# jenicek/mdir

Measured on AMD Instinct MI355X. Metric: queries/sec, exact full ranking (rOxford5k+1M-distractor shape, 2048-d fp32); mAP-medium alongside, higher is better.
Workload: dtype f32

## Files before the change

mdir_amd/csrc/mdx_rank.hip:

```cpp
#include <atomic>

#include "mdx_common.h"

#ifndef MDX_SORT_NT
#define MDX_SORT_NT 1
#endif

namespace mdx {

#ifndef MDX_SORT_ITEMS
#define MDX_SORT_ITEMS 8
#endif
constexpr int SORT_ITEMS = MDX_SORT_ITEMS;
#ifndef MDX_SORT_WAVES
#define MDX_SORT_WAVES 8
#endif
constexpr int SORT_WAVES = MDX_SORT_WAVES;
constexpr int SORT_THREADS = 64 * SORT_WAVES;
constexpr int SORT_TILE = SORT_THREADS * SORT_ITEMS;
constexpr int SUB_TILE = 64 * SORT_ITEMS;
constexpr int RADIX = 256;

__device__ __forceinline__ void bitonic_sort_lds(uint64_t *buf, int P, int tid, int nthreads)
{
    for (int size = 2; size <= P; size <<= 1)
        for (int stride = size >> 1; stride > 0; stride >>= 1) {
            for (int t = tid; t < (P >> 1); t += nthreads) {
                const int i = 2 * t - (t & (stride - 1)), j = i + stride;
                const uint64_t a = buf[i], b = buf[j];
                if ((a > b) == ((i & size) == 0)) {
                    buf[i] = b;
                    buf[j] = a;
                }
            }
            __syncthreads();
        }
}

enum { FMT_SCORES = 0, FMT_KV = 1, FMT_A = 2, FMT_B = 3, FMT_C = 4, FMT_RANKS = 5 };

constexpr int MAX_SEG = 32;
struct NoSeg { static constexpr bool HAS = false; };
struct SegTable {
    static constexpr bool HAS = true;
    const float *p[MAX_SEG];
    int64_t start[MAX_SEG + 1];
    int nseg;
    uint32_t inv_w;
};

struct SegHit { const float *p; int64_t s0, s1; int g; };

__device__ __forceinline__ SegHit seg_find(const SegTable &t, int64_t i)
{
    int g = (int)__umulhi((uint32_t)i, t.inv_w);
    if (g > t.nseg - 1) g = t.nseg - 1;
    SegHit h = {t.p[g], t.start[g], t.start[g + 1], g};
    while (i >= h.s1 && g + 1 < t.nseg) { ++g; h.p = t.p[g]; h.s0 = h.s1; h.s1 = t.start[g + 1]; }
    while (i < h.s0 && g > 0) { --g; h.p = t.p[g]; h.s1 = h.s0; h.s0 = t.start[g]; }
    h.g = g;
    return h;
}

struct SegPair { const uint32_t *a, *b; int64_t cut; bool ok; };

__device__ __forceinline__ SegPair seg_pair(const SegTable &t, const SegHit &h, int64_t q, int64_t tile_end)
{
    SegPair r = {nullptr, nullptr, h.s1, false};
    if (h.g + 1 >= t.nseg) return r;
    const int64_t n0 = t.start[h.g + 1], n1 = t.start[h.g + 2];
    if (tile_end > n1) return r;
    r.a = (const uint32_t *)(h.p + q * (h.s1 - h.s0) - h.s0);
    r.b = (const uint32_t *)(t.p[h.g + 1] + q * (n1 - n0) - n0);
    r.ok = true;
    return r;
}

__device__ __forceinline__ const float *seg_elem(const SegTable &t, int64_t q, int64_t i)
{
    const SegHit h = seg_find(t, i);
    return h.p + q * (h.s1 - h.s0) + (i - h.s0);
}

constexpr int HIST_COPIES = 8;

template <int SRC, typename SEGT = NoSeg>
__global__ __launch_bounds__(SORT_THREADS) void sort_hist_kernel(const float *__restrict__ scores,
                                                                 const void *__restrict__ src, int64_t n,
                                                                 int64_t stride, int nblk, int shift,
                                                                 uint32_t *__restrict__ block_hist, SEGT seg)
{
    static_assert(SORT_ITEMS == 8, "a lane takes 8 elements of a tile");
    constexpr bool FIRST = SRC == FMT_SCORES;
    __shared__ uint32_t h[HIST_COPIES][RADIX + 1];
    const int tid = threadIdx.x, copy = tid & (HIST_COPIES - 1);
    const int64_t q = FIRST ? (int64_t)gridDim.y - 1 - blockIdx.y : (int64_t)blockIdx.y;
    const int64_t b0 = FIRST ? (int64_t)gridDim.x - 1 - blockIdx.x : (int64_t)blockIdx.x;
    for (int e = tid; e < HIST_COPIES * (RADIX + 1); e += SORT_THREADS) (&h[0][0])[e] = 0;
    uint32_t d[SORT_ITEMS];
    int64_t first[2];
    if (SRC == FMT_A || SRC == FMT_B) {
        const int64_t i = b0 * SORT_TILE + tid * 8;
        first[0] = i;
        first[1] = i + 4;
        if (SRC == FMT_A) {
            typedef uint16_t u16x8 __attribute__((ext_vector_type(8)));
            u16x8 w = {0, 0, 0, 0, 0, 0, 0, 0};
            if (i < n) w = *(const u16x8 *)((const uint16_t *)src + q * stride + i);
#pragma unroll
            for (int j = 0; j < 8; ++j) d[j] = w[j] & 255u;
        } else {
            typedef uint8_t u8x8 __attribute__((ext_vector_type(8)));
            u8x8 w = {0, 0, 0, 0, 0, 0, 0, 0};
            if (i < n) w = *(const u8x8 *)((const uint8_t *)src + q * stride + i);
#pragma unroll
            for (int j = 0; j < 8; ++j) d[j] = w[j];
        }
    } else {
        typedef uint32_t u32x4u __attribute__((ext_vector_type(4), aligned(4)));
        const uint32_t *p = FIRST ? (const uint32_t *)scores + q * n : (const uint32_t *)src + q * stride;
        u32x4u w[2];
#pragma unroll
        for (int v = 0; v < 2; ++v) {
            first[v] = b0 * SORT_TILE + (v * SORT_THREADS + tid) * 4;
            w[v] = u32x4u{0u, 0u, 0u, 0u};
        }
        bool straddles = false;
        const int64_t tile_end = (b0 + 1) * SORT_TILE < n ? (b0 + 1) * SORT_TILE : n;
        SegHit h = {nullptr, 0, 0, 0};
        if constexpr (FIRST && SEGT::HAS) {
            h = seg_find(seg, b0 * SORT_TILE);
            straddles = tile_end > h.s1;
            p = (const uint32_t *)(h.p + q * (h.s1 - h.s0) - h.s0);
        }
        if (straddles) {
            if constexpr (SEGT::HAS) {
                const SegPair pr = seg_pair(seg, h, q, tile_end);
                if (pr.ok) {
#pragma unroll
                    for (int v = 0; v < 2; ++v) {
                        const int64_t i0 = first[v];
                        if (i0 + 4 <= pr.cut) w[v] = *(const u32x4u *)(pr.a + i0);
                        else if (i0 >= pr.cut && i0 + 4 <= tile_end) w[v] = *(const u32x4u *)(pr.b + i0);
                        else {
#pragma unroll
                            for (int j = 0; j < 4; ++j)
                                if (i0 + j < tile_end) w[v][j] = (i0 + j < pr.cut ? pr.a : pr.b)[i0 + j];
                        }
                    }
                } else {
#pragma unroll
                    for (int v = 0; v < 2; ++v)
#pragma unroll
                        for (int j = 0; j < 4; ++j)
                            if (first[v] + j < n) w[v][j] = *(const uint32_t *)seg_elem(seg, q, first[v] + j);
                }
            }
        } else if ((b0 + 1) * SORT_TILE <= n) {
#pragma unroll
            for (int v = 0; v < 2; ++v) w[v] = *(const u32x4u *)(p + first[v]);
        } else {
#pragma unroll
            for (int v = 0; v < 2; ++v)
#pragma unroll
                for (int j = 0; j < 4; ++j)
                    if (first[v] + j < n) w[v][j] = p[first[v] + j];
        }
#pragma unroll
        for (int v = 0; v < 2; ++v)
#pragma unroll
            for (int j = 0; j < 4; ++j) d[v * 4 + j] = ((FIRST ? desc_key(__uint_as_float(w[v][j])) : w[v][j]) >> shift) & 255u;
    }
    __syncthreads();
#pragma unroll
    for (int r = 0; r < SORT_ITEMS; ++r)
        if (first[r / 4] + (r % 4) < n) atomicAdd(&h[copy][d[r]], 1u);
    __syncthreads();
    for (int e = tid; e < RADIX; e += SORT_THREADS) {
        uint32_t tot = 0;
#pragma unroll
        for (int w = 0; w < HIST_COPIES; ++w) tot += h[w][e];
        block_hist[(q * nblk + b0) * RADIX + e] = tot;
    }
}

constexpr int SCAN_GROUPS = 32, SCAN_DIGITS = 32;

__global__ __launch_bounds__(SCAN_GROUPS * SCAN_DIGITS) void sort_scan_kernel(uint32_t *__restrict__ block_hist,
                                                                              int nblk,
                                                                              uint32_t *__restrict__ digit_tot)
{
    __shared__ uint32_t part[SCAN_GROUPS][SCAN_DIGITS + 1];
    const int dl = threadIdx.x & (SCAN_DIGITS - 1), g = threadIdx.x / SCAN_DIGITS;
    const int d = blockIdx.x * SCAN_DIGITS + dl;
    const int64_t q = blockIdx.y;
    const int per = (nblk + SCAN_GROUPS - 1) / SCAN_GROUPS;
    const int b0 = g * per < nblk ? g * per : nblk, b1 = (b0 + per) < nblk ? (b0 + per) : nblk;
    uint32_t *p = block_hist + q * nblk * RADIX + d;
    uint32_t sum = 0;
    constexpr int KEEP = 8;
    uint32_t kept[KEEP];
    const bool keep = per <= KEEP;
    if (keep) {
#pragma unroll
        for (int u = 0; u < KEEP; ++u) {
            kept[u] = (b0 + u) < b1 ? p[(int64_t)(b0 + u) * RADIX] : 0u;
            sum += kept[u];
        }
    } else {
        for (int b = b0; b < b1; ++b) sum += p[(int64_t)b * RADIX];
    }
    part[g][dl] = sum;
    __syncthreads();
    uint32_t run = 0;
    for (int k = 0; k < g; ++k) run += part[k][dl];
    if (g == SCAN_GROUPS - 1) digit_tot[q * RADIX + d] = run + sum;
    if (keep) {
#pragma unroll
        for (int u = 0; u < KEEP; ++u)
            if ((b0 + u) < b1) {
                p[(int64_t)(b0 + u) * RADIX] = run;
                run += kept[u];
            }
        return;
    }
    int b = b0;
    for (; b + 8 <= b1; b += 8) {
        uint32_t c[8];
#pragma unroll
        for (int u = 0; u < 8; ++u) c[u] = p[(int64_t)(b + u) * RADIX];
#pragma unroll
        for (int u = 0; u < 8; ++u) {
            p[(int64_t)(b + u) * RADIX] = run;
            run += c[u];
        }
    }
    for (; b < b1; ++b) {
        const uint32_t c = p[(int64_t)b * RADIX];
        p[(int64_t)b * RADIX] = run;
        run += c;
    }
}

template <int IN, int OUT, bool ARANK, typename SEGT = NoSeg>
__global__ __launch_bounds__(SORT_THREADS, (SORT_WAVES >= 16 ? 8 : (3 * SORT_WAVES) / 4)) void sort_scatter_kernel(
    const float *__restrict__ scores, const uint32_t *__restrict__ w_in, const void *__restrict__ h_in,
    uint32_t *__restrict__ w_out, void *__restrict__ h_out, int64_t *__restrict__ ranks,
    float *__restrict__ top_scores, int64_t n, int64_t stride, int nblk, int shift,
    const uint32_t *__restrict__ block_hist, const uint32_t *__restrict__ digit_tot, int64_t id_offset,
    int64_t klimit, SEGT seg)
{
    constexpr bool FIRST = IN == FMT_SCORES, LAST = OUT == FMT_RANKS;
    constexpr bool VAL_IN_KEY = IN == FMT_C;
    __shared__ uint32_t dtot[RADIX];
    __shared__ uint32_t wcnt[SORT_WAVES][RADIX];
    __shared__ uint32_t gdelta[RADIX];
    __shared__ uint32_t scan[RADIX];
    __shared__ uint32_t skey[SORT_TILE];
    __shared__ uint32_t sval[SORT_TILE];
    const int tid = threadIdx.x, lane = tid & 63, wave = tid >> 6;
    const int64_t q = FIRST ? (int64_t)blockIdx.y : (int64_t)gridDim.y - 1 - blockIdx.y;
    int64_t b = blockIdx.x;
#ifndef MDX_SORT_NO_XCD
    {
        const int qn = nblk / 8, rn = nblk % 8, x = (int)(blockIdx.x % 8), k = (int)(blockIdx.x / 8);
        b = (x < rn ? (int64_t)x * (qn + 1) : (int64_t)rn * (qn + 1) + (int64_t)(x - rn) * qn) + k;
    }
#endif
    if (!FIRST) b = (int64_t)nblk - 1 - b;
    for (int e = tid; e < SORT_WAVES * RADIX; e += SORT_THREADS) (&wcnt[0][0])[e] = 0;
    __syncthreads();

    const int64_t base = q * n;
    const int64_t row = q * stride;
    const int64_t tile0 = b * SORT_TILE;
    const int tile_n = (int)((n - tile0) < SORT_TILE ? (n - tile0) : SORT_TILE);
    const int sub = wave * SUB_TILE + lane;
    uint32_t key[SORT_ITEMS], val[SORT_ITEMS], pos[SORT_ITEMS];
    uint32_t gbase = 0, qtot = 0;
    if (tid < RADIX) {
        gbase = block_hist[(q * nblk + b) * RADIX + tid];
        qtot = digit_tot[q * RADIX + tid];
    }
    if (FIRST) {
        typedef uint32_t u32x4u __attribute__((ext_vector_type(4), aligned(4)));
        const uint32_t *src = (const uint32_t *)scores + base + tile0;
        bool straddles = false;
        SegHit sh = {nullptr, 0, 0, 0};
        if constexpr (SEGT::HAS) {
            sh = seg_find(seg, tile0);
            straddles = tile0 + tile_n > sh.s1;
            src = (const uint32_t *)(sh.p + q * (sh.s1 - sh.s0) + (tile0 - sh.s0));
        }
        if (straddles) {
            if constexpr (SEGT::HAS) {
                const SegPair pr = seg_pair(seg, sh, q, tile0 + tile_n);
                if (pr.ok) {
                    const uint32_t *pa = pr.a + tile0, *pb = pr.b + tile0;
                    const int cut = (int)(pr.cut - tile0);
                    for (int e = tid; e < tile_n; e += SORT_THREADS) skey[e] = desc_key(__uint_as_float((e < cut ? pa : pb)[e]));
                } else {
                    for (int e = tid; e < tile_n; e += SORT_THREADS) skey[e] = desc_key(*seg_elem(seg, q, tile0 + e));
                }
            }
        } else if (tile_n == SORT_TILE) {
            u32x4u w[SORT_ITEMS / 4];
#pragma unroll
            for (int v = 0; v < SORT_ITEMS / 4; ++v) w[v] = *(const u32x4u *)(src + (v * SORT_THREADS + tid) * 4);
#pragma unroll
            for (int v = 0; v < SORT_ITEMS / 4; ++v)
#pragma unroll
                for (int j = 0; j < 4; ++j) skey[(v * SORT_THREADS + tid) * 4 + j] = desc_key(__uint_as_float(w[v][j]));
        } else {
            for (int e = tid; e < tile_n; e += SORT_THREADS) skey[e] = desc_key(__uint_as_float(src[e]));
        }
        __syncthreads();
#pragma unroll
        for (int r = 0; r < SORT_ITEMS; ++r) {
            key[r] = (sub + r * 64) < tile_n ? skey[sub + r * 64] : 0xFFFFFFFFu;
            val[r] = (uint32_t)tile0 + (uint32_t)(sub + r * 64);
        }
    } else {
        const uint32_t *wt = w_in + row + tile0;
        const uint8_t *ht = (const uint8_t *)h_in + (row + tile0) * (IN == FMT_KV ? 4 : IN == FMT_A ? 2 : 1);
        uint32_t w[SORT_ITEMS], hh[SORT_ITEMS];
#pragma unroll
        for (int r = 0; r < SORT_ITEMS; ++r) {
            const int e = min(sub + r * 64, tile_n - 1);
            w[r] = wt[e];
            hh[r] = 0;
            if (IN == FMT_KV) hh[r] = ((const uint32_t *)ht)[e];
            if (IN == FMT_A) hh[r] = ((const uint16_t *)ht)[e];
            if (IN == FMT_B) hh[r] = ht[e];
        }
#pragma unroll
        for (int r = 0; r < SORT_ITEMS; ++r) {
            const bool valid = (sub + r * 64) < tile_n;
            if (IN == FMT_KV) {
                key[r] = valid ? w[r] : 0xFFFFFFFFu;
                val[r] = hh[r];
            } else {
                const uint32_t k = IN == FMT_C ? w[r] : ((w[r] & 0xFF000000u) | (hh[r] << (IN == FMT_A ? 8 : 16)));
                key[r] = valid ? k : 0xFFFFFFFFu;
                val[r] = w[r] & 0x00FFFFFFu;
            }
        }
    }
    if (tid < RADIX) {
        gdelta[tid] = gbase;
        dtot[tid] = qtot;
    }
    uint32_t *mycnt = wcnt[wave];
    if (ARANK) {
#pragma unroll
        for (int r = 0; r < SORT_ITEMS; ++r) {
            pos[r] = 0;
            if ((sub + r * 64) < tile_n)
                pos[r] = __hip_atomic_fetch_add(&mycnt[(key[r] >> shift) & 255u], 1u, __ATOMIC_RELAXED,
                                                __HIP_MEMORY_SCOPE_WORKGROUP);
        }
    } else {
#pragma unroll
        for (int r = 0; r < SORT_ITEMS; ++r) {
            const bool valid = (sub + r * 64) < tile_n;
            const uint32_t d = (key[r] >> shift) & 255u;
            uint32_t dlo = 0, dhi = 0;
#pragma unroll
            for (int bit = 0; bit < 8; ++bit) {
                int32_t sel = __builtin_amdgcn_sbfe((int32_t)d, bit, 1);
                asm("" : "+v"(sel));
                const uint64_t m = __builtin_amdgcn_ballot_w64(sel < 0);
                dlo = __builtin_amdgcn_bitop3_b32(dlo, (uint32_t)m, (uint32_t)sel, 0xF6);
                dhi = __builtin_amdgcn_bitop3_b32(dhi, (uint32_t)(m >> 32), (uint32_t)sel, 0xF6);
            }
            const uint64_t vmask = __builtin_amdgcn_ballot_w64(valid);
            const uint32_t plo = (uint32_t)vmask & ~dlo, phi = (uint32_t)(vmask >> 32) & ~dhi;
            const uint32_t rank = __builtin_amdgcn_mbcnt_hi(phi, __builtin_amdgcn_mbcnt_lo(plo, 0u));
            const uint32_t cnt = __popc(plo) + __popc(phi);
            const uint32_t old = mycnt[d];
            __builtin_amdgcn_wave_barrier();
            if (valid && rank == 0) mycnt[d] = old + cnt;
            __builtin_amdgcn_wave_barrier();
            pos[r] = old + rank;
        }
    }
    __syncthreads();
    if (tid < RADIX) {
        uint32_t run = 0;
#pragma unroll
        for (int w = 0; w < SORT_WAVES; ++w) {
            const uint32_t c = wcnt[w][tid];
            wcnt[w][tid] = run;
            run += c;
        }
        scan[tid] = run;
    }
    __syncthreads();
    if (wave == 0) {
        const uint32_t t0 = scan[4 * lane], t1 = scan[4 * lane + 1], t2 = scan[4 * lane + 2],
                       t3 = scan[4 * lane + 3];
        const uint32_t g0 = dtot[4 * lane], g1 = dtot[4 * lane + 1], g2 = dtot[4 * lane + 2],
                       g3 = dtot[4 * lane + 3];
        const uint32_t mine = t0 + t1 + t2 + t3, gmine = g0 + g1 + g2 + g3;
        const uint32_t inc = wave_inclusive_sum(mine), ginc = wave_inclusive_sum(gmine);
        const uint32_t ex = inc - mine, gex = ginc - gmine;
        const uint32_t toff[4] = {ex, ex + t0, ex + t0 + t1, ex + t0 + t1 + t2};
        const uint32_t goff[4] = {gex, gex + g0, gex + g0 + g1, gex + g0 + g1 + g2};
#pragma unroll
        for (int k = 0; k < 4; ++k) {
            const int dgt = 4 * lane + k;
            scan[dgt] = toff[k];
            gdelta[dgt] += goff[k] - toff[k];
        }
    }
    __syncthreads();
#pragma unroll
    for (int r = 0; r < SORT_ITEMS; ++r) {
        if ((sub + r * 64) >= tile_n) continue;
        const uint32_t d = (key[r] >> shift) & 255u;
        const uint32_t lp = scan[d] + mycnt[d] + pos[r];
        skey[lp] = key[r];
        if (!VAL_IN_KEY) sval[lp] = val[r];
    }
    __syncthreads();
    constexpr bool OFF32 = IN == FMT_C;
    char *const wrow = (char *)(w_out + row), *const hrow = (char *)h_out + row * (OUT == FMT_KV ? 4 : OUT == FMT_A ? 2 : 1);
#pragma unroll
    for (int r = 0; r < SORT_ITEMS; ++r) {
        const int i = r * SORT_THREADS + tid;
        if (i >= tile_n) continue;
        const uint32_t k = skey[i], v = VAL_IN_KEY ? (k & 0x00FFFFFFu) : sval[i];
        const uint32_t dst32 = gdelta[(k >> shift) & 255u] + (uint32_t)i;
        if (LAST) {
            const int64_t dst = (int64_t)dst32;
            if (dst < klimit) {
                if (ranks) {
                    int64_t *dstp = OFF32 ? (int64_t *)((char *)(ranks + q * klimit) + (dst32 << 3)) : ranks + q * klimit + dst;
#if MDX_SORT_NT
                    __builtin_nontemporal_store((int64_t)v + id_offset, dstp);
#else
                    *dstp = (int64_t)v + id_offset;
#endif
                }
                if (top_scores) top_scores[q * klimit + dst] = scores[base + v];
            }
        } else if (OUT == FMT_KV) {
            w_out[row + (int64_t)dst32] = k;
            ((uint32_t *)h_out)[row + (int64_t)dst32] = v;
        } else {
            *(uint32_t *)(wrow + (dst32 << 2)) = (k & 0xFF000000u) | v;
            if (OUT == FMT_A) *(uint16_t *)(hrow + (dst32 << 1)) = (uint16_t)(k >> 8);
            if (OUT == FMT_B) *(uint8_t *)(hrow + dst32) = (uint8_t)(k >> 16);
        }
    }
}

constexpr int CNT_TILE = 4096;
constexpr int CNT_ITEMS = CNT_TILE / 256;

constexpr int CNTB_REFS = 256;

__global__ __launch_bounds__(256) void rank_count_bsearch_kernel(
    const float *__restrict__ scores, int64_t n, int64_t id_offset,
    const float *__restrict__ ref_scores, const int64_t *__restrict__ ref_ids,
    const int64_t *__restrict__ offsets, unsigned long long *__restrict__ cnt, int nblk)
{
    constexpr int CNT_COPIES = 8;
    __shared__ uint64_t sref[CNTB_REFS];
    __shared__ uint32_t histc[CNT_COPIES][CNTB_REFS + 1];
    __shared__ uint32_t hist[CNTB_REFS + 1];
    __shared__ uint32_t wsum[4];
    const int tid = threadIdx.x, lane = tid & 63, copy = tid & (CNT_COPIES - 1);
    const int64_t q = blockIdx.y;
    const int64_t lo = offsets[q], hi = offsets[q + 1];
    for (int64_t r0 = lo; r0 < hi; r0 += CNTB_REFS) {
        const int nref = (int)((hi - r0) < CNTB_REFS ? (hi - r0) : CNTB_REFS);
        int P = 2;
        while (P < nref) P <<= 1;
        __syncthreads();
        uint64_t mine = ~0ull;
        if (tid < nref) {
            const int64_t id = ref_ids[r0 + tid];
            const uint32_t idc = id < 0 ? 0u : (id > 0xFFFFFFFFll ? 0xFFFFFFFFu : (uint32_t)id);
            mine = ((uint64_t)desc_key(ref_scores[r0 + tid]) << 32) | idc;
        }
        sref[tid] = mine;
        for (int e = tid; e < CNT_COPIES * (CNTB_REFS + 1); e += 256) (&histc[0][0])[e] = 0;
        __syncthreads();
        bitonic_sort_lds(sref, CNTB_REFS, tid, 256);
        for (int b = blockIdx.x; b < nblk; b += gridDim.x) {
            const int64_t t0 = (int64_t)b * CNT_TILE;
            uint64_t el[CNT_ITEMS];
            typedef uint32_t u32x4u __attribute__((ext_vector_type(4), aligned(4)));
            const uint32_t *row = (const uint32_t *)scores + q * n;
            if (t0 + CNT_TILE <= n) {
                u32x4u w[CNT_ITEMS / 4];
#pragma unroll
                for (int v = 0; v < CNT_ITEMS / 4; ++v) w[v] = *(const u32x4u *)(row + t0 + (v * 256 + tid) * 4);
#pragma unroll
                for (int v = 0; v < CNT_ITEMS / 4; ++v)
#pragma unroll
                    for (int j = 0; j < 4; ++j) {
                        const int64_t i = t0 + (v * 256 + tid) * 4 + j;
                        el[v * 4 + j] = ((uint64_t)desc_key(__uint_as_float(w[v][j])) << 32) | (uint32_t)(i + id_offset);
                    }
            } else {
#pragma unroll
                for (int e = 0; e < CNT_ITEMS; ++e) {
                    const int64_t i = t0 + (e / 4 * 256 + tid) * 4 + e % 4;
                    el[e] = i < n ? ((uint64_t)desc_key(scores[q * n + i]) << 32) | (uint32_t)(i + id_offset) : ~0ull;
                }
            }
            const uint64_t last = sref[nref - 1];
#pragma unroll
            for (int e = 0; e < CNT_ITEMS; ++e) {
                const bool live = el[e] < last;
                if (__ballot(live) == 0) continue;
                uint32_t u = 0;
                for (int step = P >> 1; step > 0; step >>= 1)
                    u += (sref[u + step - 1] <= el[e]) ? (uint32_t)step : 0u;
                if (live) atomicAdd(&histc[copy][u], 1u);
            }
        }
        __syncthreads();
        uint32_t inc = 0;
#pragma unroll
        for (int c = 0; c < CNT_COPIES; ++c) inc += histc[c][tid];
#pragma unroll
        for (int o = 1; o < 64; o <<= 1) {
            const uint32_t v = __shfl_up(inc, o, 64);
            if (lane >= o) inc += v;
        }
        if (lane == 63) wsum[tid >> 6] = inc;
        __syncthreads();
        for (int w = 0; w < (tid >> 6); ++w) inc += wsum[w];
        __syncthreads();
        hist[tid] = inc;
        __syncthreads();
        if (tid < nref) {
            uint32_t pos = 0;
            for (int step = CNTB_REFS >> 1; step > 0; step >>= 1)
                pos += (sref[pos + step - 1] < mine) ? (uint32_t)step : 0u;
            const uint32_t v = hist[pos];
            if (v) atomicAdd(&cnt[r0 + tid], (unsigned long long)v);
        }
    }
}

__global__ void gather_scores_kernel(const float *__restrict__ scores, int64_t n, int64_t nq,
                                     const int64_t *__restrict__ ids,
                                     const int64_t *__restrict__ offsets, int64_t total,
                                     float *__restrict__ out)
{
    const int64_t t = (int64_t)blockIdx.x * blockDim.x + threadIdx.x;
    if (t >= total) return;
    int64_t a = 0, b = nq;
    while (b - a > 1) {
        const int64_t m = (a + b) >> 1;
        if (offsets[m] <= t) a = m; else b = m;
    }
    const int64_t id = ids[t];
    out[t] = (id >= 0 && id < n) ? scores[a * n + id] : __uint_as_float(0x7FC00000u);
}

struct RankWs {
    uint32_t *w[2];
    void *h[2];
    uint32_t *block_hist;
    uint32_t *digit_tot;
    int nblk;
    int64_t stride;
};

static int64_t carve(RankWs *ws, char *base, int64_t n, int64_t nq)
{
    const int64_t nblk = ceil_div(n, SORT_TILE);
    const int64_t stride = round_up(n, 256);
    const int64_t elems = stride * nq * 4;
    int64_t off = 0;
    for (int i = 0; i < 2; ++i) {
        if (ws) ws->w[i] = (uint32_t *)(base + off);
        off += elems;
        if (ws) ws->h[i] = (void *)(base + off);
        off += elems;
    }
    if (ws) ws->block_hist = (uint32_t *)(base + off);
    off += round_up(nq * nblk * RADIX * 4, 256);
    if (ws) ws->digit_tot = (uint32_t *)(base + off);
    off += round_up(nq * RADIX * 4, 256);
    if (ws) ws->nblk = (int)nblk;
    if (ws) ws->stride = stride;
    return off;
}

constexpr int LS_THREADS = 512, LS_WAVES = LS_THREADS / 64, LS_MAX_ITEMS = 16, LS_CAP = LS_THREADS * LS_MAX_ITEMS;

struct LsShared {
    uint32_t key[LS_CAP];
    uint32_t val[LS_CAP];
    uint32_t cnt[LS_WAVES][RADIX];
    uint32_t tot[RADIX];
    uint32_t diff;
};

template <int ITEMS>
__device__ __forceinline__ void lds_radix_sort(uint32_t (&key)[ITEMS], uint32_t (&val)[ITEMS], int m, LsShared &sh)
{
    const int tid = threadIdx.x, lane = tid & 63, wave = tid >> 6;
    const int sub = wave * 64 * ITEMS + lane;
    uint32_t pos[ITEMS];
    uint32_t diff = 0;
    if (tid == 0) {
        sh.diff = 0;
        sh.tot[0] = key[0];
    }
    uint32_t *mycnt = sh.cnt[wave];
#pragma unroll
    for (int e = 0; e < RADIX / 64; ++e) mycnt[e * 64 + lane] = 0;
    __syncthreads();
    const uint32_t first = sh.tot[0];
#pragma unroll
    for (int r = 0; r < ITEMS; ++r)
        if (sub + r * 64 < m) diff |= key[r] ^ first;
#pragma unroll
    for (int o = 32; o > 0; o >>= 1) diff |= __shfl_xor(diff, o, 64);
    if (lane == 0 && diff) atomicOr(&sh.diff, diff);
    __syncthreads();
    diff = sh.diff;
    bool staged = false;
    for (int pass = 0; pass < 4; ++pass) {
        const int shift = 8 * pass;
        if (((diff >> shift) & 255u) == 0) continue;
#pragma unroll
        for (int r = 0; r < ITEMS; ++r) {
            pos[r] = 0;
            if (sub + r * 64 < m)
                pos[r] = __hip_atomic_fetch_add(&mycnt[(key[r] >> shift) & 255u], 1u, __ATOMIC_RELAXED, __HIP_MEMORY_SCOPE_WORKGROUP);
        }
        __syncthreads();
        if (wave == 0) {
            uint32_t t[4], c[4][LS_WAVES];
#pragma unroll
            for (int k = 0; k < 4; ++k)
#pragma unroll
                for (int w = 0; w < LS_WAVES; ++w) c[k][w] = sh.cnt[w][64 * k + lane];
#pragma unroll
            for (int k = 0; k < 4; ++k) {
                uint32_t run = 0;
#pragma unroll
                for (int w = 0; w < LS_WAVES; ++w) {
                    sh.cnt[w][64 * k + lane] = run;
                    run += c[k][w];
                }
                t[k] = run;
            }
            uint32_t inc[4] = {t[0], t[1], t[2], t[3]};
#pragma unroll
            for (int o = 1; o < 64; o <<= 1)
#pragma unroll
                for (int k = 0; k < 4; ++k) {
                    const uint32_t v = __shfl_up(inc[k], o, 64);
                    if (lane >= o) inc[k] += v;
                }
            uint32_t before = 0;
#pragma unroll
            for (int k = 0; k < 4; ++k) {
                sh.tot[64 * k + lane] = before + inc[k] - t[k];
                before += __shfl(inc[k], 63, 64);
            }
        }
        __syncthreads();
#pragma unroll
        for (int r = 0; r < ITEMS; ++r) {
            if (sub + r * 64 >= m) continue;
            const uint32_t d = (key[r] >> shift) & 255u;
            const uint32_t dst = sh.tot[d] + mycnt[d] + pos[r];
            sh.key[dst] = key[r];
            sh.val[dst] = val[r];
        }
        staged = true;
        if ((diff >> shift) >> 8) {
#pragma unroll
            for (int e = 0; e < RADIX / 64; ++e) mycnt[e * 64 + lane] = 0;
            __syncthreads();
#pragma unroll
            for (int r = 0; r < ITEMS; ++r)
                if (sub + r * 64 < m) {
                    key[r] = sh.key[sub + r * 64];
                    val[r] = sh.val[sub + r * 64];
                }
        } else {
            __syncthreads();
        }
    }
    if (!staged) {
#pragma unroll
        for (int r = 0; r < ITEMS; ++r)
            if (sub + r * 64 < m) {
                sh.key[sub + r * 64] = key[r];
                sh.val[sub + r * 64] = val[r];
            }
        __syncthreads();
    }
}

template <int ITEMS>
__device__ __forceinline__ void rank_small(const float *__restrict__ scores, const SegTable &seg, int64_t q, int n, int64_t id_offset,
                                           int64_t *__restrict__ ranks, float *__restrict__ top_scores, int klimit, LsShared &sh)
{
    const int tid = threadIdx.x, lane = tid & 63, wave = tid >> 6;
    const int sub = wave * 64 * ITEMS + lane;
    uint32_t key[ITEMS], val[ITEMS];
    const float *row = scores + q * (int64_t)n;
#pragma unroll
    for (int r = 0; r < ITEMS; ++r) {
        const int i = sub + r * 64;
        const int j = i < n ? i : n - 1;
        key[r] = desc_key(seg.nseg > 0 ? *seg_elem(seg, q, j) : row[j]);
        val[r] = (uint32_t)j;
    }
    lds_radix_sort<ITEMS>(key, val, n, sh);
    for (int i = tid; i < klimit; i += LS_THREADS) {
        const uint32_t v = sh.val[i];
        if (ranks) ranks[q * (int64_t)klimit + i] = (int64_t)v + id_offset;
        if (top_scores) top_scores[q * (int64_t)klimit + i] = seg.nseg > 0 ? *seg_elem(seg, q, v) : row[v];
    }
}

__global__ __launch_bounds__(LS_THREADS, 2) void rank_small_kernel(const float *__restrict__ scores, SegTable seg, int n, int64_t id_offset,
                                                                   int64_t *__restrict__ ranks, float *__restrict__ top_scores, int klimit)
{
    __shared__ LsShared sh;
    const int64_t q = blockIdx.x;
    if (n <= LS_THREADS * 4) rank_small<4>(scores, seg, q, n, id_offset, ranks, top_scores, klimit, sh);
    else if (n <= LS_THREADS * 8) rank_small<8>(scores, seg, q, n, id_offset, ranks, top_scores, klimit, sh);
    else if (n <= LS_THREADS * 12) rank_small<12>(scores, seg, q, n, id_offset, ranks, top_scores, klimit, sh);
    else rank_small<16>(scores, seg, q, n, id_offset, ranks, top_scores, klimit, sh);
}

__global__ __launch_bounds__(SORT_THREADS) void lds_order_probe_kernel(uint32_t seed, int *bad)
{
    __shared__ uint32_t cnt[SORT_WAVES][RADIX];
    const int tid = threadIdx.x, lane = tid & 63, wave = tid >> 6;
    for (int e = tid; e < SORT_WAVES * RADIX; e += SORT_THREADS) (&cnt[0][0])[e] = 0;
    __syncthreads();
    uint32_t x = seed ^ (uint32_t)(tid * 2654435761u) ^ (blockIdx.x * 40503u);
    int wrong = 0;
    for (int round = 0; round < 64; ++round) {
        x = x * 1664525u + 1013904223u;
        const int mode = (round + blockIdx.x) % 3;
        const uint32_t d = mode == 0 ? (x >> 24) : mode == 1 ? ((x >> 24) & 3u) * 37u : 200u;
        const bool active = ((x >> 8) & 15u) != 0;
        uint32_t before = 0, got = 0;
        if (active) {
            before = cnt[wave][d];
            __builtin_amdgcn_wave_barrier();
            got = __hip_atomic_fetch_add(&cnt[wave][d], 1u, __ATOMIC_RELAXED, __HIP_MEMORY_SCOPE_WORKGROUP);
        }
        uint32_t lower = 0;
        for (int l = 0; l < 64; ++l) {
            const uint32_t dl = __shfl(d, l, 64);
            const bool al = __shfl(active ? 1 : 0, l, 64) != 0;
            if (al && dl == d && l < lane) ++lower;
        }
        if (active && got != before + lower) wrong = 1;
        __builtin_amdgcn_wave_barrier();
    }
    if (wrong) atomicOr(bad, 1);
}

static std::atomic<int> g_arank[64];

int probe_lds_order(hipStream_t s)
{
    int dev = 0;
    if (hipGetDevice(&dev) != hipSuccess || dev < 0 || dev >= 64) return 1;
    int known = g_arank[dev].load(std::memory_order_acquire);
    if (known > 0) return known;
    hipStreamCaptureStatus cap = hipStreamCaptureStatusNone;
    if (hipStreamIsCapturing(s, &cap) != hipSuccess || cap != hipStreamCaptureStatusNone) return 0;
    int verdict = 1;
    hipDeviceProp_t prop;
    if (hipGetDeviceProperties(&prop, dev) == hipSuccess && !strncmp(prop.gcnArchName, "gfx950", 6)) {
        int *bad = nullptr, host = 1;
        if (hipMalloc(&bad, sizeof(int)) == hipSuccess) {
            bool ok = hipMemsetAsync(bad, 0, sizeof(int), s) == hipSuccess;
            if (ok) {
                hipLaunchKernelGGL(lds_order_probe_kernel, dim3(1024), dim3(SORT_THREADS), 0, s, 0x9E3779B9u, bad);
                ok = hipMemcpyAsync(&host, bad, sizeof(int), hipMemcpyDeviceToHost, s) == hipSuccess &&
                     hipStreamSynchronize(s) == hipSuccess;
            }
            (void)hipFree(bad);
            if (ok && host == 0) verdict = 2;
        }
    }
    g_arank[dev].store(verdict, std::memory_order_release);
    return verdict;
}

static int forced_rank_form()
{
    static const char *force = getenv("MDX_SORT_RANK");
    if (force && !strcmp(force, "ballot")) return 0;
    if (force && !strcmp(force, "atomic")) return 1;
    return -1;
}

static bool atomic_rank_ok(hipStream_t s)
{
    const int forced = forced_rank_form();
    if (forced >= 0) return forced == 1;
    return probe_lds_order(s) == 2;
}

static bool atomic_rank_known()
{
    const int forced = forced_rank_form();
    if (forced >= 0) return forced == 1;
    int dev = 0;
    if (hipGetDevice(&dev) != hipSuccess || dev < 0 || dev >= 64) return false;
    return g_arank[dev].load(std::memory_order_acquire) == 2;
}

static int rank_route(int64_t n, bool arank)
{
    static const bool no_pack = getenv("MDX_SORT_NO_PACK") && atoi(getenv("MDX_SORT_NO_PACK")) != 0;
    static const bool no_small = getenv("MDX_SORT_SMALL") && atoi(getenv("MDX_SORT_SMALL")) == 0;
    if (arank && n <= LS_CAP && !no_small) return MDX_RANK_ROUTE_SMALL;
    if (n <= (1ll << 24) && !no_pack) return MDX_RANK_ROUTE_PACKED;
    return MDX_RANK_ROUTE_KV;
}

template <int IN, int OUT, typename SEGT>
static void sort_pass_on(const RankWs &ws, const float *scores, int64_t n, int64_t nq, int pass, int64_t id_offset,
                         int64_t *ranks, float *top_scores, int64_t klimit, bool arank, const SEGT &seg, hipStream_t s)
{
    const int shift = 8 * pass;
    const uint32_t *w_in = pass == 0 ? nullptr : ws.w[(pass - 1) & 1];
    const void *h_in = pass == 0 ? nullptr : ws.h[(pass - 1) & 1];
    const dim3 grid((unsigned)ws.nblk, (unsigned)nq), blk(SORT_THREADS);
    const void *digits = (IN == FMT_A || IN == FMT_B) ? h_in : (const void *)w_in;
    hipLaunchKernelGGL((sort_hist_kernel<IN, SEGT>), grid, blk, 0, s, scores, digits, n, ws.stride, ws.nblk, shift,
                       ws.block_hist, seg);
    hipLaunchKernelGGL(sort_scan_kernel, dim3(RADIX / SCAN_DIGITS, (unsigned)nq), dim3(SCAN_GROUPS * SCAN_DIGITS), 0, s,
                       ws.block_hist, ws.nblk, ws.digit_tot);
    if (arank)
        hipLaunchKernelGGL((sort_scatter_kernel<IN, OUT, true, SEGT>), grid, blk, 0, s, scores, w_in, h_in, ws.w[pass & 1],
                           ws.h[pass & 1], ranks, top_scores, n, ws.stride, ws.nblk, shift, ws.block_hist, ws.digit_tot,
                           id_offset, klimit, seg);
    else
        hipLaunchKernelGGL((sort_scatter_kernel<IN, OUT, false, SEGT>), grid, blk, 0, s, scores, w_in, h_in, ws.w[pass & 1],
                           ws.h[pass & 1], ranks, top_scores, n, ws.stride, ws.nblk, shift, ws.block_hist, ws.digit_tot,
                           id_offset, klimit, seg);
}

template <int IN, int OUT>
static void sort_pass(const RankWs &ws, const float *scores, int64_t n, int64_t nq, int pass, int64_t id_offset,
                      int64_t *ranks, float *top_scores, int64_t klimit, bool arank, const SegTable &seg, hipStream_t s)
{
    if (IN == FMT_SCORES && seg.nseg > 0)
        sort_pass_on<IN, OUT, SegTable>(ws, scores, n, nq, pass, id_offset, ranks, top_scores, klimit, arank, seg, s);
    else
        sort_pass_on<IN, OUT, NoSeg>(ws, scores, n, nq, pass, id_offset, ranks, top_scores, klimit, arank, NoSeg{}, s);
}

static int rank_impl(const float *scores, int64_t n, int64_t nq, int64_t id_offset, int64_t *ranks,
                     float *top_scores, int64_t klimit, void *workspace, int64_t workspace_bytes,
                     hipStream_t s, const char *who, const SegTable *segments = nullptr)
{
    SegTable seg;
    if (segments) seg = *segments;
    else memset(&seg, 0, sizeof seg);
    if (seg.nseg > 0) {
        const uint64_t w = (uint64_t)ceil_div(n, (int64_t)seg.nseg), inv = (1ull << 32) / (w ? w : 1);
        seg.inv_w = inv > 0xFFFFFFFFull ? 0xFFFFFFFFu : (uint32_t)inv;
    }
    MDX_CHECK_ARG(scores || seg.nseg > 0, "%s: NULL scores", who);
    MDX_CHECK_ARG(n > 0 && nq > 0, "%s: n=%lld nq=%lld must be positive", who, (long long)n,
                  (long long)nq);
    MDX_CHECK_ARG(n < (1ll << 32) && nq < 65536, "%s: n or nq too large", who);
    const int64_t need = carve(nullptr, nullptr, n, nq);
    MDX_CHECK_WORKSPACE(who, workspace, workspace_bytes, need);
    RankWs ws;
    carve(&ws, (char *)workspace, n, nq);
    const bool arank = atomic_rank_ok(s);
    const int route = rank_route(n, arank);
    if (route == MDX_RANK_ROUTE_SMALL) {
        hipLaunchKernelGGL(rank_small_kernel, dim3((unsigned)nq), dim3(LS_THREADS), 0, s, scores, seg, (int)n, id_offset, ranks, top_scores,
                           (int)klimit);
        MDX_LAUNCH_CHECK();
        return MDX_OK;
    }
    if (route == MDX_RANK_ROUTE_PACKED) {
        sort_pass<FMT_SCORES, FMT_A>(ws, scores, n, nq, 0, id_offset, ranks, top_scores, klimit, arank, seg, s);
        sort_pass<FMT_A, FMT_B>(ws, scores, n, nq, 1, id_offset, ranks, top_scores, klimit, arank, seg, s);
        sort_pass<FMT_B, FMT_C>(ws, scores, n, nq, 2, id_offset, ranks, top_scores, klimit, arank, seg, s);
        sort_pass<FMT_C, FMT_RANKS>(ws, scores, n, nq, 3, id_offset, ranks, top_scores, klimit, arank, seg, s);
    } else {
        sort_pass<FMT_SCORES, FMT_KV>(ws, scores, n, nq, 0, id_offset, ranks, top_scores, klimit, arank, seg, s);
        sort_pass<FMT_KV, FMT_KV>(ws, scores, n, nq, 1, id_offset, ranks, top_scores, klimit, arank, seg, s);
        sort_pass<FMT_KV, FMT_KV>(ws, scores, n, nq, 2, id_offset, ranks, top_scores, klimit, arank, seg, s);
        sort_pass<FMT_KV, FMT_RANKS>(ws, scores, n, nq, 3, id_offset, ranks, top_scores, klimit, arank, seg, s);
    }
    MDX_LAUNCH_CHECK();
    return MDX_OK;
}

struct SelState { uint32_t prefix, mask, k_rem, resolved; };

constexpr int SEL_CAP = 4096;

__global__ __launch_bounds__(SORT_THREADS) void select_hist_kernel(const float *__restrict__ scores, int64_t n,
                                                                   int nblk, int shift,
                                                                   const SelState *__restrict__ st,
                                                                   uint32_t *__restrict__ block_hist)
{
    __shared__ uint32_t h[SORT_WAVES / 2][RADIX];
    const int tid = threadIdx.x, wave = tid >> 6;
    const int64_t q = blockIdx.y;
    const SelState s = st[q];
    if (s.resolved) return;
    for (int64_t b = blockIdx.x; b < nblk; b += gridDim.x) {
        for (int e = tid; e < (SORT_WAVES / 2) * RADIX; e += SORT_THREADS) (&h[0][0])[e] = 0;
        uint32_t k[SORT_ITEMS];
        bool ok[SORT_ITEMS];
        if ((b + 1) * SORT_TILE <= n) {
            typedef uint32_t u32x4u __attribute__((ext_vector_type(4), aligned(4)));
            const uint32_t *row = (const uint32_t *)scores + q * n + b * SORT_TILE;
            u32x4u w[SORT_ITEMS / 4];
#pragma unroll
            for (int v = 0; v < SORT_ITEMS / 4; ++v) w[v] = *(const u32x4u *)(row + (v * SORT_THREADS + tid) * 4);
#pragma unroll
            for (int r = 0; r < SORT_ITEMS; ++r) {
                k[r] = desc_key(__uint_as_float(w[r / 4][r % 4]));
                ok[r] = true;
            }
        } else {
#pragma unroll
            for (int r = 0; r < SORT_ITEMS; ++r) {
                const int64_t i = b * SORT_TILE + r * SORT_THREADS + tid;
                ok[r] = i < n;
                k[r] = ok[r] ? desc_key(scores[q * n + i]) : 0u;
            }
        }
        __syncthreads();
#pragma unroll
        for (int r = 0; r < SORT_ITEMS; ++r)
            if (ok[r] && (k[r] & s.mask) == s.prefix) atomicAdd(&h[wave >> 1][(k[r] >> shift) & 255u], 1u);
        __syncthreads();
        if (tid < RADIX) {
            uint32_t tot = 0;
#pragma unroll
            for (int w = 0; w < SORT_WAVES / 2; ++w) tot += h[w][tid];
            block_hist[(q * nblk + b) * RADIX + tid] = tot;
        }
        __syncthreads();
    }
}

__global__ __launch_bounds__(1024) void select_step_kernel(const uint32_t *__restrict__ block_hist, int nblk,
                                                           int shift, SelState *__restrict__ st,
                                                           uint32_t *__restrict__ tile_less,
                                                           uint32_t *__restrict__ tile_eq)
{
    __shared__ uint32_t part[4][RADIX];
    __shared__ uint32_t cum[RADIX];
    __shared__ uint32_t dstar_s;
    const int tid = threadIdx.x, d = tid & 255, g = tid >> 8;
    const int64_t q = blockIdx.x;
    SelState s = st[q];
    if (s.resolved) return;
    const uint32_t *bh = block_hist + q * nblk * RADIX;
    const int per = (nblk + 3) / 4, b0 = g * per, b1 = (b0 + per) < nblk ? (b0 + per) : nblk;
    uint32_t tot = 0;
    for (int b = b0; b < b1; ++b) tot += bh[(int64_t)b * RADIX + d];
    part[g][d] = tot;
    __syncthreads();
    if (g == 0) cum[d] = part[0][d] + part[1][d] + part[2][d] + part[3][d];
    __syncthreads();
    for (int off = 1; off < RADIX; off <<= 1) {
        const uint32_t v = (g == 0 && d >= off) ? cum[d - off] : 0u;
        __syncthreads();
        if (g == 0) cum[d] += v;
        __syncthreads();
    }
    if (g == 0 && cum[d] >= s.k_rem && (d == 0 || cum[d - 1] < s.k_rem)) dstar_s = d;
    __syncthreads();
    const uint32_t ds = dstar_s;
    const uint32_t c_eq = ds == 0 ? cum[0] : cum[ds] - cum[ds - 1];
    const uint32_t c_less = cum[ds] - c_eq;
    const int lane = tid & 63, wv = tid >> 6;
    for (int b = wv; b < nblk; b += 16) {
        const uint4 c = *(const uint4 *)(bh + (int64_t)b * RADIX + 4 * lane);
        const uint32_t e0 = 4 * lane;
        uint32_t less = (e0 < ds ? c.x : 0u) + (e0 + 1 < ds ? c.y : 0u) + (e0 + 2 < ds ? c.z : 0u) + (e0 + 3 < ds ? c.w : 0u);
#pragma unroll
        for (int o = 32; o > 0; o >>= 1) less += __shfl_xor(less, o, 64);
        if (lane == 0) {
            tile_less[q * nblk + b] += less;
            tile_eq[q * nblk + b] = bh[(int64_t)b * RADIX + ds];
        }
    }
    if (tid == 0) {
        s.prefix |= ds << shift;
        s.mask |= 255u << shift;
        s.k_rem -= c_less;
        s.resolved = (shift == 0 || c_eq <= s.k_rem + SEL_CAP) ? 1u : 0u;
        st[q] = s;
    }
}

__global__ __launch_bounds__(256) void select_offsets_kernel(uint32_t *__restrict__ tile_less,
                                                             uint32_t *__restrict__ tile_eq, int nblk)
{
    __shared__ uint32_t sa[256], sb[256];
    __shared__ uint32_t carry_a, carry_b;
    const int t = threadIdx.x;
    const int64_t q = blockIdx.x;
    uint32_t *la = tile_less + q * nblk, *lb = tile_eq + q * nblk;
    if (t == 0) { carry_a = 0; carry_b = 0; }
    __syncthreads();
    uint32_t part = 0;
    for (int b = t; b < nblk; b += 256) part += la[b];
    sa[t] = part;
    __syncthreads();
    for (int off = 128; off > 0; off >>= 1) { if (t < off) sa[t] += sa[t + off]; __syncthreads(); }
    const uint32_t total_less = sa[0];
    __syncthreads();
    for (int b0 = 0; b0 < nblk; b0 += 256) {
        const int b = b0 + t;
        const uint32_t va = b < nblk ? la[b] : 0u, vb = b < nblk ? lb[b] : 0u;
        sa[t] = va; sb[t] = vb;
        __syncthreads();
        for (int off = 1; off < 256; off <<= 1) {
            const uint32_t xa = t >= off ? sa[t - off] : 0u, xb = t >= off ? sb[t - off] : 0u;
            __syncthreads();
            sa[t] += xa; sb[t] += xb;
            __syncthreads();
        }
        if (b < nblk) { la[b] = carry_a + sa[t] - va; lb[b] = total_less + carry_b + sb[t] - vb; }
        __syncthreads();
        if (t == 255) { carry_a += sa[255]; carry_b += sb[255]; }
        __syncthreads();
    }
}

__global__ __launch_bounds__(SORT_THREADS) void select_scatter_kernel(const float *__restrict__ scores, int64_t n,
                                                                      int nblk, const SelState *__restrict__ st,
                                                                      const uint32_t *__restrict__ off_less,
                                                                      const uint32_t *__restrict__ off_eq,
                                                                      uint32_t cap_total,
                                                                      float *__restrict__ cand_scores,
                                                                      uint32_t *__restrict__ cand_ids)
{
    __shared__ uint32_t wl[SORT_WAVES], we[SORT_WAVES];
    const int tid = threadIdx.x, lane = tid & 63, wave = tid >> 6;
    const int64_t q = blockIdx.y, b = blockIdx.x;
    const SelState s = st[q];
    const int64_t sub0 = b * SORT_TILE + wave * SUB_TILE;
    float v[SORT_ITEMS];
    uint32_t pl[SORT_ITEMS], pe[SORT_ITEMS];
    uint32_t nl = 0, ne = 0;
    const uint64_t lt_mask = (1ull << lane) - 1ull;
#pragma unroll
    for (int r = 0; r < SORT_ITEMS; ++r) {
        const int64_t i = sub0 + r * 64 + lane;
        v[r] = i < n ? scores[q * n + i] : 0.0f;
    }
#pragma unroll
    for (int r = 0; r < SORT_ITEMS; ++r) {
        const int64_t i = sub0 + r * 64 + lane;
        const uint32_t km = desc_key(v[r]) & s.mask;
        const bool is_l = i < n && km < s.prefix, is_e = i < n && km == s.prefix;
        const uint64_t ml = __ballot(is_l), me = __ballot(is_e);
        pl[r] = is_l ? nl + __popcll(ml & lt_mask) : 0xFFFFFFFFu;
        pe[r] = is_e ? ne + __popcll(me & lt_mask) : 0xFFFFFFFFu;
        nl += __popcll(ml);
        ne += __popcll(me);
    }
    if (lane == 0) { wl[wave] = nl; we[wave] = ne; }
    __syncthreads();
    uint32_t bl = off_less[q * nblk + b], be = off_eq[q * nblk + b];
    for (int w = 0; w < wave; ++w) { bl += wl[w]; be += we[w]; }
#pragma unroll
    for (int r = 0; r < SORT_ITEMS; ++r) {
        const uint32_t pos = pl[r] != 0xFFFFFFFFu ? bl + pl[r] : (pe[r] != 0xFFFFFFFFu ? be + pe[r] : 0xFFFFFFFFu);
        if (pos < cap_total) {
            cand_scores[q * cap_total + pos] = v[r];
            cand_ids[q * cap_total + pos] = (uint32_t)(sub0 + r * 64 + lane);
        }
    }
}

__global__ void select_init_kernel(SelState *st, int64_t nq, uint32_t k)
{
    const int64_t q = (int64_t)blockIdx.x * blockDim.x + threadIdx.x;
    if (q < nq) st[q] = SelState{0u, 0u, k, 0u};
}

__global__ void select_gather_kernel(const int64_t *__restrict__ local, const float *__restrict__ cand_scores,
                                     const uint32_t *__restrict__ cand_ids, int64_t nq, int64_t k,
                                     uint32_t cap_total, int64_t id_offset, int64_t *__restrict__ top_ids,
                                     float *__restrict__ top_scores)
{
    const int64_t t = (int64_t)blockIdx.x * blockDim.x + threadIdx.x;
    if (t >= nq * k) return;
    const int64_t q = t / k, j = local[t];
    if (top_ids) top_ids[t] = (int64_t)cand_ids[q * cap_total + j] + id_offset;
    if (top_scores) top_scores[t] = cand_scores[q * cap_total + j];
}

struct SelWs {
    uint32_t *block_hist, *tile_less, *tile_eq, *cand_ids;
    SelState *state;
    float *cand_scores;
    int64_t *local;
    char *sort_ws;
    int64_t sort_ws_bytes;
};

static int64_t carve_select(SelWs *ws, char *base, int64_t n, int64_t nq, int64_t k)
{
    const int64_t nblk = ceil_div(n, SORT_TILE), ct = k + SEL_CAP;
    int64_t off = 0;
    auto take = [&](int64_t bytes) { char *p = base ? base + off : nullptr; off += round_up(bytes, 256); return p; };
    char *p;
    p = take(nq * nblk * RADIX * 4); if (ws) ws->block_hist = (uint32_t *)p;
    p = take(nq * nblk * 4);         if (ws) ws->tile_less = (uint32_t *)p;
    p = take(nq * nblk * 4);         if (ws) ws->tile_eq = (uint32_t *)p;
    p = take(nq * sizeof(SelState)); if (ws) ws->state = (SelState *)p;
    p = take(nq * ct * 4);           if (ws) ws->cand_scores = (float *)p;
    p = take(nq * ct * 4);           if (ws) ws->cand_ids = (uint32_t *)p;
    p = take(nq * k * 8);            if (ws) ws->local = (int64_t *)p;
    const int64_t sw = carve(nullptr, nullptr, ct, nq);
    p = take(sw);                    if (ws) { ws->sort_ws = p; ws->sort_ws_bytes = sw; }
    return off;
}

static int topk_select(const float *scores, int64_t n, int64_t nq, int64_t k, int64_t id_offset,
                       int64_t *top_ids, float *top_scores, void *workspace, hipStream_t s)
{
    SelWs ws;
    carve_select(&ws, (char *)workspace, n, nq, k);
    const int nblk = (int)ceil_div(n, SORT_TILE);
    const uint32_t ct = (uint32_t)(k + SEL_CAP);
// ... 487 lines not shown
```

Before: 19920.

## Shrink scatter LDS with 16-bit staged values and halve FMT_B histogram threads

In scatter passes that write packed outputs, the LDS value staging buffer drops from 32-bit to 16-bit entries. Pass 0 stores tile-local indices, and later passes fold the low 8 bits of the value into the already-consumed key byte. Launch bounds request higher minimum occupancy for those packed rank kernels. The byte-digit histogram kernel uses half the threads, each loading 16 bytes. The aim is less LDS and higher occupancy in the scatter kernel plus wider loads in the histogram, at the cost of relying on the key's low byte being zero after the shift, which adds correctness risk.

```diff
diff --git a/mdir_amd/csrc/mdx_rank.hip b/mdir_amd/csrc/mdx_rank.hip
--- a/mdir_amd/csrc/mdx_rank.hip
+++ b/mdir_amd/csrc/mdx_rank.hip
@@ -84,37 +84,40 @@
 
 constexpr int HIST_COPIES = 8;
 
+constexpr int hist_threads(int src) { return src == FMT_B ? SORT_THREADS / 2 : SORT_THREADS; }
+
 template <int SRC, typename SEGT = NoSeg>
-__global__ __launch_bounds__(SORT_THREADS) void sort_hist_kernel(const float *__restrict__ scores,
+__global__ __launch_bounds__(hist_threads(SRC)) void sort_hist_kernel(const float *__restrict__ scores,
                                                                  const void *__restrict__ src, int64_t n,
                                                                  int64_t stride, int nblk, int shift,
                                                                  uint32_t *__restrict__ block_hist, SEGT seg)
 {
     static_assert(SORT_ITEMS == 8, "a lane takes 8 elements of a tile");
     constexpr bool FIRST = SRC == FMT_SCORES;
+    constexpr int THREADS = hist_threads(SRC), ITEMS = SORT_TILE / THREADS;
     __shared__ uint32_t h[HIST_COPIES][RADIX + 1];
     const int tid = threadIdx.x, copy = tid & (HIST_COPIES - 1);
     const int64_t q = FIRST ? (int64_t)gridDim.y - 1 - blockIdx.y : (int64_t)blockIdx.y;
     const int64_t b0 = FIRST ? (int64_t)gridDim.x - 1 - blockIdx.x : (int64_t)blockIdx.x;
-    for (int e = tid; e < HIST_COPIES * (RADIX + 1); e += SORT_THREADS) (&h[0][0])[e] = 0;
-    uint32_t d[SORT_ITEMS];
-    int64_t first[2];
+    for (int e = tid; e < HIST_COPIES * (RADIX + 1); e += THREADS) (&h[0][0])[e] = 0;
+    uint32_t d[ITEMS];
+    int64_t first[ITEMS / 4];
     if (SRC == FMT_A || SRC == FMT_B) {
-        const int64_t i = b0 * SORT_TILE + tid * 8;
-        first[0] = i;
-        first[1] = i + 4;
-        if (SRC == FMT_A) {
+        const int64_t i = b0 * SORT_TILE + tid * ITEMS;
+#pragma unroll
+        for (int v = 0; v < ITEMS / 4; ++v) first[v] = i + 4 * v;
+        if constexpr (SRC == FMT_A) {
             typedef uint16_t u16x8 __attribute__((ext_vector_type(8)));
             u16x8 w = {0, 0, 0, 0, 0, 0, 0, 0};
             if (i < n) w = *(const u16x8 *)((const uint16_t *)src + q * stride + i);
 #pragma unroll
             for (int j = 0; j < 8; ++j) d[j] = w[j] & 255u;
-        } else {
-            typedef uint8_t u8x8 __attribute__((ext_vector_type(8)));
-            u8x8 w = {0, 0, 0, 0, 0, 0, 0, 0};
-            if (i < n) w = *(const u8x8 *)((const uint8_t *)src + q * stride + i);
-#pragma unroll
-            for (int j = 0; j < 8; ++j) d[j] = w[j];
+        } else if constexpr (SRC == FMT_B) {
+            typedef uint8_t u8x16 __attribute__((ext_vector_type(16)));
+            u8x16 w = {0, 0, 0, 0, 0, 0, 0, 0, 0, 0, 0, 0, 0, 0, 0, 0};
+            if (i < n) w = *(const u8x16 *)((const uint8_t *)src + q * stride + i);
+#pragma unroll
+            for (int j = 0; j < 16; ++j) d[j] = w[j];
         }
     } else {
         typedef uint32_t u32x4u __attribute__((ext_vector_type(4), aligned(4)));
@@ -173,10 +176,10 @@
     }
     __syncthreads();
 #pragma unroll
-    for (int r = 0; r < SORT_ITEMS; ++r)
+    for (int r = 0; r < ITEMS; ++r)
         if (first[r / 4] + (r % 4) < n) atomicAdd(&h[copy][d[r]], 1u);
     __syncthreads();
-    for (int e = tid; e < RADIX; e += SORT_THREADS) {
+    for (int e = tid; e < RADIX; e += THREADS) {
         uint32_t tot = 0;
 #pragma unroll
         for (int w = 0; w < HIST_COPIES; ++w) tot += h[w][e];
@@ -242,8 +245,17 @@
     }
 }
 
+template <bool SHORT> struct SortVal { typedef uint32_t type; };
+template <> struct SortVal<true> { typedef uint16_t type; };
+
+constexpr int scatter_min_waves(int out, bool arank)
+{
+    const bool packed = out == FMT_A || out == FMT_B || out == FMT_C;
+    return SORT_WAVES >= 16 || (SORT_WAVES == 8 && packed && arank) ? 8 : (3 * SORT_WAVES) / 4;
+}
+
 template <int IN, int OUT, bool ARANK, typename SEGT = NoSeg>
-__global__ __launch_bounds__(SORT_THREADS, (SORT_WAVES >= 16 ? 8 : (3 * SORT_WAVES) / 4)) void sort_scatter_kernel(
+__global__ __launch_bounds__(SORT_THREADS, scatter_min_waves(OUT, ARANK)) void sort_scatter_kernel(
     const float *__restrict__ scores, const uint32_t *__restrict__ w_in, const void *__restrict__ h_in,
     uint32_t *__restrict__ w_out, void *__restrict__ h_out, int64_t *__restrict__ ranks,
     float *__restrict__ top_scores, int64_t n, int64_t stride, int nblk, int shift,
@@ -252,12 +264,15 @@
 {
     constexpr bool FIRST = IN == FMT_SCORES, LAST = OUT == FMT_RANKS;
     constexpr bool VAL_IN_KEY = IN == FMT_C;
+    constexpr bool VAL16 = OUT == FMT_A || OUT == FMT_B || OUT == FMT_C;
+    constexpr bool LOW8_IN_KEY = VAL16 && !FIRST;
+    static_assert(!VAL16 || SORT_TILE <= 65536, "the tile-local index of pass 0 is staged in 16 bits");
     __shared__ uint32_t dtot[RADIX];
     __shared__ uint32_t wcnt[SORT_WAVES][RADIX];
     __shared__ uint32_t gdelta[RADIX];
     __shared__ uint32_t scan[RADIX];
     __shared__ uint32_t skey[SORT_TILE];
-    __shared__ uint32_t sval[SORT_TILE];
+    __shared__ typename SortVal<VAL16>::type sval[SORT_TILE];
     const int tid = threadIdx.x, lane = tid & 63, wave = tid >> 6;
     const int64_t q = FIRST ? (int64_t)blockIdx.y : (int64_t)gridDim.y - 1 - blockIdx.y;
     int64_t b = blockIdx.x;
@@ -318,7 +333,7 @@
 #pragma unroll
         for (int r = 0; r < SORT_ITEMS; ++r) {
             key[r] = (sub + r * 64) < tile_n ? skey[sub + r * 64] : 0xFFFFFFFFu;
-            val[r] = (uint32_t)tile0 + (uint32_t)(sub + r * 64);
+            val[r] = (VAL16 ? 0u : (uint32_t)tile0) + (uint32_t)(sub + r * 64);
         }
     } else {
         const uint32_t *wt = w_in + row + tile0;
@@ -419,8 +434,8 @@
         if ((sub + r * 64) >= tile_n) continue;
         const uint32_t d = (key[r] >> shift) & 255u;
         const uint32_t lp = scan[d] + mycnt[d] + pos[r];
-        skey[lp] = key[r];
-        if (!VAL_IN_KEY) sval[lp] = val[r];
+        skey[lp] = LOW8_IN_KEY ? (key[r] | (val[r] & 255u)) : key[r];
+        if (!VAL_IN_KEY) sval[lp] = (typename SortVal<VAL16>::type)(LOW8_IN_KEY ? val[r] >> 8 : val[r]);
     }
     __syncthreads();
     constexpr bool OFF32 = IN == FMT_C;
@@ -429,7 +444,10 @@
     for (int r = 0; r < SORT_ITEMS; ++r) {
         const int i = r * SORT_THREADS + tid;
         if (i >= tile_n) continue;
-        const uint32_t k = skey[i], v = VAL_IN_KEY ? (k & 0x00FFFFFFu) : sval[i];
+        const uint32_t k = skey[i];
+        const uint32_t v = VAL_IN_KEY ? (k & 0x00FFFFFFu)
+                         : LOW8_IN_KEY ? (((uint32_t)sval[i] << 8) | (k & 255u))
+                         : VAL16 ? (uint32_t)tile0 + sval[i] : (uint32_t)sval[i];
         const uint32_t dst32 = gdelta[(k >> shift) & 255u] + (uint32_t)i;
         if (LAST) {
             const int64_t dst = (int64_t)dst32;
@@ -840,7 +858,7 @@
     const void *h_in = pass == 0 ? nullptr : ws.h[(pass - 1) & 1];
     const dim3 grid((unsigned)ws.nblk, (unsigned)nq), blk(SORT_THREADS);
     const void *digits = (IN == FMT_A || IN == FMT_B) ? h_in : (const void *)w_in;
-    hipLaunchKernelGGL((sort_hist_kernel<IN, SEGT>), grid, blk, 0, s, scores, digits, n, ws.stride, ws.nblk, shift,
+    hipLaunchKernelGGL((sort_hist_kernel<IN, SEGT>), grid, dim3(hist_threads(IN)), 0, s, scores, digits, n, ws.stride, ws.nblk, shift,
                        ws.block_hist, seg);
     hipLaunchKernelGGL(sort_scan_kernel, dim3(RADIX / SCAN_DIGITS, (unsigned)nq), dim3(SCAN_GROUPS * SCAN_DIGITS), 0, s,
                        ws.block_hist, ws.nblk, ws.digit_tot);
```

Result: faster. 20180, median of 6 (+1.3%).
